# frosinastojanovska/image-captioning

Measured on AMD Instinct MI355X. Metric: captions/sec (train step) on 1024px x 32RoI x 15tok synth, higher is better.
Workload: dtype f32 (split-bf16x3 products, fp32 accumulate: 73 of 85 conv layers on the bf16 pipe, the rest and the decoder exact fp32 MFMA); 1 GPU; BASELINE configs[2] (configs[3] at 8 GPUs): frozen ResNet-101+FPN fwd + PyramidROIAlign + RoI head + v2-inject decoder fwd/bwd + AMSGrad, 1024x1024 synth images, 32 RoI/img, 15-token captions, V=10000; backbone=resnet101, images_per_gpu=2, global_batch_images=2, parallelism=dp1, stage4_blocks=22, pipeline=encoder(i+1) || decoder(i), 2 HIP streams, rccl_ranks=1

## Files before the change

### image-captioning_amd/csrc/conv_wino.hip

```cpp
#include "igemm_bf16s.h"
#include <algorithm>

namespace dcap {
namespace wino {

constexpr int NTHREADS = 256;

struct Args {
    const float* x;
    const f4* u;
    float* y;
    const float* scale;
    const float* shift;
    int N, H, W, Cin, Cout, relu;
    int gy, gx, groups;
    unsigned x_bytes, u_bytes;
};

__global__ void wino_pack_kernel(const float* __restrict__ w, float* __restrict__ u, int Cin, int Cout) {
    const long total = (long)Cin * Cout;
    const int NTG = Cout / 32, KC = Cin / 16;
    for (long idx = (long)blockIdx.x * blockDim.x + threadIdx.x; idx < total; idx += (long)gridDim.x * blockDim.x) {
        const int cin = (int)(idx % Cin), cout = (int)(idx / Cin);
        float g[3][3];
#pragma unroll
        for (int t = 0; t < 9; ++t) g[t / 3][t % 3] = w[((long)cout * 9 + t) * Cin + cin];
        float gg[4][3];
#pragma unroll
        for (int c = 0; c < 3; ++c) {
            gg[0][c] = g[0][c];
            gg[1][c] = 0.5f * (g[0][c] + g[1][c] + g[2][c]);
            gg[2][c] = 0.5f * (g[0][c] - g[1][c] + g[2][c]);
            gg[3][c] = g[2][c];
        }
        const int ntg = cout >> 5, i = cout & 31, kc = cin >> 4, kk = cin & 15, h = kk >> 3, j = (kk & 7) >> 2, e = kk & 3;
#pragma unroll
        for (int a = 0; a < 4; ++a) {
            const float r[4] = {gg[a][0], 0.5f * (gg[a][0] + gg[a][1] + gg[a][2]), 0.5f * (gg[a][0] - gg[a][1] + gg[a][2]), gg[a][2]};
#pragma unroll
            for (int b = 0; b < 4; ++b) {
                const int xi = 4 * a + b;
                u[((((long)(xi * NTG + ntg) * KC + kc) * 2 + j) * 64 + (h * 32 + i)) * 4 + e] = r[b];
            }
        }
    }
}

__global__ void wino_pack_b3_kernel(const float* __restrict__ w, unsigned short* __restrict__ u, int Cin, int Cout) {
    const long total = (long)Cin * Cout;
    const int NTG = Cout / 32, KC = Cin / 16;
    for (long idx = (long)blockIdx.x * blockDim.x + threadIdx.x; idx < total; idx += (long)gridDim.x * blockDim.x) {
        const int cin = (int)(idx % Cin), cout = (int)(idx / Cin);
        float g[3][3];
#pragma unroll
        for (int t = 0; t < 9; ++t) g[t / 3][t % 3] = w[((long)cout * 9 + t) * Cin + cin];
        float gg[4][3];
#pragma unroll
        for (int c = 0; c < 3; ++c) {
            gg[0][c] = g[0][c];
            gg[1][c] = 0.5f * (g[0][c] + g[1][c] + g[2][c]);
            gg[2][c] = 0.5f * (g[0][c] - g[1][c] + g[2][c]);
            gg[3][c] = g[2][c];
        }
        const int ntg = cout >> 5, i = cout & 31, kc = cin >> 4, kk = cin & 15, h = kk >> 3, jj = kk & 7;
#pragma unroll
        for (int a = 0; a < 4; ++a) {
            const float r[4] = {gg[a][0], 0.5f * (gg[a][0] + gg[a][1] + gg[a][2]), 0.5f * (gg[a][0] - gg[a][1] + gg[a][2]), gg[a][2]};
#pragma unroll
            for (int b = 0; b < 4; ++b) {
                const int xi = 4 * a + b;
                float x = r[b];
#pragma unroll
                for (int piece = 0; piece < 3; ++piece) {
                    const unsigned short pb = __builtin_bit_cast(unsigned short, (__bf16)x);
                    x -= __uint_as_float((unsigned)pb << 16);
                    u[((((long)(xi * NTG + ntg) * KC + kc) * 3 + piece) * 64 + (h * 32 + i)) * 8 + jj] = pb;
                }
            }
        }
    }
}

__device__ __forceinline__ unsigned img32_addr(int xi, int tile, int chunk) {
    return (unsigned)((((xi * 32 + tile) << 3) + (chunk ^ ((tile >> 1) & 7))) << 4);
}
__device__ __forceinline__ void bt_cols(const f4 (&t)[4], f4 (&v)[4]) {
    v[0] = t[0] - t[2];
    v[1] = t[1] + t[2];
    v[2] = t[2] - t[1];
    v[3] = t[1] - t[3];
}

namespace wp {
constexpr int PW = 18, NDMA = 6;
__device__ __forceinline__ int patch_index(int y, int x) { return y * PW + (x >> 1) + (PW / 2) * (x & 1); }
__device__ __forceinline__ int patch_swizzle(int y, int x) { return ((x >> 2) & 1) | (((y >> 1) & 3) << 1); }
template <int HALVES>
struct Cfg {
    static constexpr int NT = 256 * HALVES, TGY = 4 * HALVES, TGX = 8, PH = 2 * TGY + 2, NPIX = PH * PW, SLOTS = NPIX * 8;
    static constexpr int BUF = 32768 * HALVES;
    static constexpr int LDS_BYTES = 2 * BUF;
    static_assert(NDMA * NT >= SLOTS && NDMA * NT * 16 <= BUF, "patch buffer; the kernel issues the pieces three per step");
};
}

typedef unsigned u32x4 __attribute__((ext_vector_type(4)));

__device__ __forceinline__ void split8(const f4& va, const f4& vb, u32x4& p0, u32x4& p1, u32x4& p2) {
    unsigned a0, a1, a2, b0, b1, b2, c0, c1, c2, d0, d1, d2;
    split_pair(va[0], va[1], a0, a1, a2);
    split_pair(va[2], va[3], b0, b1, b2);
    split_pair(vb[0], vb[1], c0, c1, c2);
    split_pair(vb[2], vb[3], d0, d1, d2);
    p0 = u32x4{a0, b0, c0, d0};
    p1 = u32x4{a1, b1, c1, d1};
    p2 = u32x4{a2, b2, c2, d2};
}
__device__ __forceinline__ f32x16 mfma_b(const u32x4& a, const u32x4& b, const f32x16& c) {
    return __builtin_amdgcn_mfma_f32_32x32x16_bf16(__builtin_bit_cast(bf16x8, a), __builtin_bit_cast(bf16x8, b), c, 0, 0, 0);
}

template <int HALVES, bool B3>
__device__ __forceinline__ void wino_body(const Args& a) {
    using namespace wp;
    typedef Cfg<HALVES> C;
    constexpr int NT64 = C::NT, SLOTS = C::SLOTS, BUF = C::BUF;
    extern __shared__ __attribute__((aligned(16))) char smem[];
    const int tid = threadIdx.x, lane = tid & 63;
    const int wave = __builtin_amdgcn_readfirstlane(tid >> 6);
    const int wa = wave & 3, th = wave >> 2;
    const int gpi = a.gy * a.gx;
    const int NTG = a.Cout >> 5, KC = a.Cin >> 4, KP = a.Cin >> 5;
    const int total = a.groups * NTG;
    const __amdgpu_buffer_rsrc_t rsrc = __builtin_amdgcn_make_buffer_rsrc(const_cast<float*>(a.x), 0, (int)a.x_bytes, 0x00020000);

    int nb, img, gyi, gxi;
    unsigned doff[NDMA];
    const f4* ubase;
    unsigned ubyte3;
    auto setup = [&](int item) {
        const int bid = xcd_remap(item, total);
        nb = bid / a.groups;
        const int g = bid - nb * a.groups;
        img = g / gpi;
        const int gr = g - img * gpi;
        gyi = gr / a.gx;
        gxi = gr - gyi * a.gx;
#pragma unroll
        for (int n = 0; n < NDMA; ++n) {
            const int s = n * NT64 + tid, pq = s >> 3, py = pq / PW, rem = pq - py * PW;
            const int px = rem < PW / 2 ? 2 * rem : 2 * (rem - PW / 2) + 1;
            const int iy = gyi * 2 * C::TGY - 1 + py, ix = gxi * 2 * C::TGX - 1 + px;
            const bool in = s < SLOTS && (unsigned)iy < (unsigned)a.H && (unsigned)ix < (unsigned)a.W;
            const int c8 = (s & 7) ^ patch_swizzle(py, px);
            doff[n] = in ? (unsigned)(((((long)img * a.H + iy) * a.W + ix) * a.Cin + 4 * c8) * 4) : kOobOffset;
        }
        ubase = a.u + lane + (((long)(4 * wa) * NTG + nb) * KC << 7);
        ubyte3 = (unsigned)((4 * wa) * NTG + nb) * (unsigned)KC * 3072u;
    };
    auto issue_dma_pieces = [&](int pair, int buf, int n0, int n1) {
#pragma unroll
        for (int n = n0; n < n1; ++n)
            __builtin_amdgcn_raw_ptr_buffer_load_lds(rsrc, (__attribute__((address_space(3))) void*)(smem + buf * BUF + (n * NT64 + wave * 64) * 16), 16,
                                                     (int)doff[n], pair * 128, 0, 0);
    };
    auto issue_dma = [&](int pair, int buf) { issue_dma_pieces(pair, buf, 0, NDMA); };
    const long ustep = (long)NTG * KC << 7;
    auto load_u_part = [&](f4 (&dst)[4][2], int kc, int b0, int b1) {
#pragma unroll
        for (int b = b0; b < b1; ++b) {
            const f4* p = ubase + b * ustep + ((long)kc << 7);
            dst[b][0] = p[0];
            dst[b][1] = p[64];
        }
    };
    auto load_u = [&](f4 (&dst)[4][2], int kc) { load_u_part(dst, kc, 0, 4); };
    const __amdgpu_buffer_rsrc_t rsrc_u = __builtin_amdgcn_make_buffer_rsrc(const_cast<f4*>(a.u), 0, (int)a.u_bytes, 0x00020000);
    const unsigned ustep3 = (unsigned)NTG * KC * 3 * 1024u;
    auto load_u3 = [&](u32x4 (&dst)[3], int kc, int b) {
        const unsigned so = __builtin_amdgcn_readfirstlane(ubyte3 + (unsigned)b * ustep3 + (unsigned)kc * 3072u);
        dst[0] = __builtin_bit_cast(u32x4, buf_f4s(rsrc_u, (unsigned)lane * 16u, so));
        dst[1] = __builtin_bit_cast(u32x4, buf_f4s(rsrc_u, (unsigned)lane * 16u, so + 1024u));
        dst[2] = __builtin_bit_cast(u32x4, buf_f4s(rsrc_u, (unsigned)lane * 16u, so + 2048u));
    };

    const int fi = lane & 31, fh = lane >> 5;
    const int tile = 32 * th + fi, tyl = tile >> 3, txl = tile & 7;
    const int r1 = (wa == 0) ? 0 : (wa == 2 ? 2 : 1), r2 = (wa == 0 || wa == 1) ? 2 : (wa == 2 ? 1 : 3);
    const float sgn = (wa == 1) ? 1.f : -1.f;
    unsigned paddr[2][4];
#pragma unroll
    for (int rr = 0; rr < 2; ++rr)
#pragma unroll
        for (int c = 0; c < 4; ++c) {
            const int py = 2 * tyl + (rr ? r2 : r1), px = 2 * txl + c;
            paddr[rr][c] = (unsigned)(patch_index(py, px) * 128 + (((2 * fh) ^ patch_swizzle(py, px)) << 4));
        }
    auto read_d = [&](f4 (&d)[2][4], int st) {
        const unsigned k = (unsigned)(((st & 1) << 4) ^ ((st >> 1) << 6));
#pragma unroll
        for (int rr = 0; rr < 2; ++rr)
#pragma unroll
            for (int c = 0; c < 4; ++c) d[rr][c] = *reinterpret_cast<const f4*>(smem + (paddr[rr][c] ^ k));
    };
    auto transform = [&](const f4 (&d)[2][4], f4 (&v)[4]) {
        f4 t[4];
#pragma unroll
        for (int c = 0; c < 4; ++c) t[c] = d[1][c] * sgn + d[0][c];
        bt_cols(t, v);
    };

    int item = blockIdx.x;
    if (item >= total) return;
    setup(item);
    issue_dma(0, 0);
    f4 ub[2][4][2];
    u32x4 u3[4][3];
    if constexpr (B3) {
#pragma unroll
        for (int b = 0; b < 4; ++b) load_u3(u3[b], 0, b);
    } else {
        load_u(ub[0], 0);
    }
    for (;;) {
        f32x16 acc[4];
#pragma unroll
        for (int b = 0; b < 4; ++b)
#pragma unroll
            for (int r = 0; r < 16; ++r) acc[b][r] = 0.f;
        auto pair = [&](int p, auto more_c) {
            constexpr bool more = decltype(more_c)::value;
            asm volatile("s_waitcnt vmcnt(0)" ::: "memory");
            __syncthreads();
            if constexpr (B3) {
                f4 dA[2][4], dB[2][4], t0[4], t1[4];
                u32x4 V[2][3];
                auto make_t = [&]() {
#pragma unroll
                    for (int c = 0; c < 4; ++c) {
                        t0[c] = dA[1][c] * sgn + dA[0][c];
                        t1[c] = dB[1][c] * sgn + dB[0][c];
                    }
                };
                auto prep = [&](u32x4 (&dst)[3], int b) {
                    const f4 va = b == 0 ? t0[0] - t0[2] : (b == 1 ? t0[1] + t0[2] : (b == 2 ? t0[2] - t0[1] : t0[1] - t0[3]));
                    const f4 vb = b == 0 ? t1[0] - t1[2] : (b == 1 ? t1[1] + t1[2] : (b == 2 ? t1[2] - t1[1] : t1[1] - t1[3]));
                    split8(va, vb, dst[0], dst[1], dst[2]);
                };
                read_d(dA, 0);
                read_d(dB, 1);
                make_t();
                prep(V[0], 0);
#pragma unroll
                for (int q = 0; q < 8; ++q) {
                    const int half = q >> 2, b = q & 3;
                    if (q == 1) read_d(dA, 2);
                    if (q == 2) read_d(dB, 3);
                    __builtin_amdgcn_sched_barrier(0);
                    if constexpr (more) if (q < NDMA) issue_dma_pieces(p + 1, (p + 1) & 1, q, q + 1);
                    const u32x4 (&vq)[3] = V[q & 1];
                    acc[b] = mfma_b(u3[b][0], vq[2], acc[b]);
                    acc[b] = mfma_b(u3[b][1], vq[1], acc[b]);
                    acc[b] = mfma_b(u3[b][2], vq[0], acc[b]);
                    acc[b] = mfma_b(u3[b][1], vq[0], acc[b]);
                    acc[b] = mfma_b(u3[b][0], vq[1], acc[b]);
                    acc[b] = mfma_b(u3[b][0], vq[0], acc[b]);
                    if (q == 3) make_t();
                    if (q < 7) prep(V[(q + 1) & 1], (q + 1) & 3);
                    load_u3(u3[b], min(2 * p + half + 1, KC - 1), b);
#pragma unroll
                    for (int m = 0; m < 6; ++m) {
                        __builtin_amdgcn_sched_group_barrier(0x008, 1, 0);
                        __builtin_amdgcn_sched_group_barrier(0x020, 1, 0);
                        if (q == 3) __builtin_amdgcn_sched_group_barrier(0x002, 15, 0);
                        else __builtin_amdgcn_sched_group_barrier(0x002, 9, 0);
                    }
                    __builtin_amdgcn_sched_barrier(0);
                }
#pragma unroll
                for (int rr = 0; rr < 2; ++rr)
#pragma unroll
                    for (int c = 0; c < 4; ++c) paddr[rr][c] ^= (unsigned)BUF;
                return;
            }
            f4 d[2][4], vcur[4], vnext[4];
            read_d(d, 0);
            transform(d, vcur);
#pragma unroll
            for (int st = 0; st < 4; ++st) {
                const int half = st >> 1, j = st & 1;
                if (st < 3) read_d(d, st + 1);
                __builtin_amdgcn_sched_barrier(0);
                if constexpr (more) if (st < 2) issue_dma_pieces(p + 1, (p + 1) & 1, 3 * st, 3 * st + 3);
                load_u_part(ub[half ^ 1], min(2 * p + half + 1, KC - 1), 2 * j, 2 * j + 2);
#pragma unroll
                for (int e = 0; e < 2; ++e)
#pragma unroll
                    for (int b = 0; b < 4; ++b) acc[b] = __builtin_amdgcn_mfma_f32_32x32x2f32(ub[half][b][j][e], vcur[b][e], acc[b], 0, 0, 0);
#pragma unroll
                for (int m = 0; m < 8; ++m) {
                    __builtin_amdgcn_sched_group_barrier(0x008, 1, 0);
                    __builtin_amdgcn_sched_group_barrier(0x020, 1, 0);
                }
                __builtin_amdgcn_sched_barrier(0);
                if (st < 3) transform(d, vnext);
#pragma unroll
                for (int e = 2; e < 4; ++e)
#pragma unroll
                    for (int b = 0; b < 4; ++b) acc[b] = __builtin_amdgcn_mfma_f32_32x32x2f32(ub[half][b][j][e], vcur[b][e], acc[b], 0, 0, 0);
                if (st < 3) {
#pragma unroll
                    for (int m = 0; m < 8; ++m) {
                        __builtin_amdgcn_sched_group_barrier(0x008, 1, 0);
                        __builtin_amdgcn_sched_group_barrier(0x002, 4, 0);
                    }
                }
                __builtin_amdgcn_sched_barrier(0);
                if (st < 3) {
#pragma unroll
                    for (int b = 0; b < 4; ++b) vcur[b] = vnext[b];
                }
            }
#pragma unroll
            for (int rr = 0; rr < 2; ++rr)
#pragma unroll
                for (int c = 0; c < 4; ++c) paddr[rr][c] ^= (unsigned)BUF;
        };
        for (int p = 0; p < KP - 1; ++p) pair(p, std::true_type{});
        pair(KP - 1, std::false_type{});
        if (KP & 1) {
#pragma unroll
            for (int rr = 0; rr < 2; ++rr)
#pragma unroll
                for (int c = 0; c < 4; ++c) paddr[rr][c] ^= (unsigned)BUF;
        }

        const int onb = nb, oimg = img, ogy = gyi, ogx = gxi;
        const int next = item + (int)gridDim.x;
        const int oq = tid & 7, ocout = onb * 32 + 4 * oq;
        f4 sc = (f4)(1.f), sh = (f4)(0.f);
        if (a.scale) sc = *reinterpret_cast<const f4*>(a.scale + ocout);
        if (a.shift) sh = *reinterpret_cast<const f4*>(a.shift + ocout);
        __syncthreads();
        if (next < total) {
            setup(next);
            issue_dma(0, 0);
            if constexpr (B3) {
#pragma unroll
                for (int b = 0; b < 4; ++b) load_u3(u3[b], 0, b);
            } else {
                load_u(ub[0], 0);
            }
        }
        {
            const f32x16 s0 = acc[0] + acc[1] + acc[2], s1 = acc[1] - acc[2] - acc[3];
#pragma unroll
            for (int gq = 0; gq < 4; ++gq) {
                const f4 m0 = {s0[4 * gq], s0[4 * gq + 1], s0[4 * gq + 2], s0[4 * gq + 3]};
                const f4 m1 = {s1[4 * gq], s1[4 * gq + 1], s1[4 * gq + 2], s1[4 * gq + 3]};
                *reinterpret_cast<f4*>(smem + BUF + th * 32768 + img32_addr(2 * wa, fi, 2 * gq + fh)) = m0;
                *reinterpret_cast<f4*>(smem + BUF + th * 32768 + img32_addr(2 * wa + 1, fi, 2 * gq + fh)) = m1;
            }
        }
        __syncthreads();
        {
            const int oth = tid >> 8, ti = (tid >> 3) & 31;
            f4 sv[4][2];
#pragma unroll
            for (int r = 0; r < 4; ++r)
#pragma unroll
                for (int qx = 0; qx < 2; ++qx) sv[r][qx] = *reinterpret_cast<const f4*>(smem + BUF + oth * 32768 + img32_addr(2 * r + qx, ti, oq));
            const int otile = 32 * oth + ti, ty = ogy * C::TGY + (otile >> 3), tx = ogx * C::TGX + (otile & 7), cout = ocout;
#pragma unroll
            for (int qx = 0; qx < 2; ++qx) {
                const f4 o[2] = {sv[0][qx] + sv[1][qx] + sv[2][qx], sv[1][qx] - sv[2][qx] - sv[3][qx]};
#pragma unroll
                for (int pr = 0; pr < 2; ++pr) {
                    f4 val = o[pr] * sc + sh;
                    if (a.relu) val = f4{fmaxf(val[0], 0.f), fmaxf(val[1], 0.f), fmaxf(val[2], 0.f), fmaxf(val[3], 0.f)};
                    if (2 * ty + pr < a.H && 2 * tx + qx < a.W)
                        *reinterpret_cast<f4*>(a.y + (((long)oimg * a.H + 2 * ty + pr) * a.W + 2 * tx + qx) * a.Cout + cout) = val;
                }
            }
        }
        if (next >= total) break;
        item = next;
    }
}

__global__ __launch_bounds__(512, 1) void wino64_kernel(Args a) { wino_body<2, false>(a); }
__global__ __launch_bounds__(256, 2) void wino32_kernel(Args a) { wino_body<1, false>(a); }
__global__ __launch_bounds__(512, 1) void wino64b_kernel(Args a) { wino_body<2, true>(a); }
__global__ __launch_bounds__(256, 2) void wino32b_kernel(Args a) { wino_body<1, true>(a); }

}

static bool wino_shape_ok(const dc_conv_desc* d, const void* u) {
    return u != nullptr && d->math == DC_MATH_F32 && d->kh == 3 && d->kw == 3 && d->stride == 1 && d->pad_t == 1 && d->pad_l == 1 &&
           d->Ho == d->H && d->Wo == d->W && d->Cin % 32 == 0 && d->Cout % 32 == 0 && d->res_mode == 0 && d->split_k <= 1 && aligned16(d->y) &&
           aligned16(u) && (!d->scale || aligned16(d->scale)) && (!d->shift || aligned16(d->shift)) &&
           (size_t)d->N * d->H * d->W * d->Cin * sizeof(float) < (1ull << 31);
}

static bool wino_b3(const dc_conv_desc* d) { return wino_shape_ok(d, d->w_wino_b3); }
bool conv_winograd_supported(const dc_conv_desc* d) { return wino_b3(d) || wino_shape_ok(d, d->w_wino); }
bool conv_winograd_split_bf16(const dc_conv_desc* d) { return wino_b3(d); }

static int wino_force() {
    static const int force = env_int("DCAP_WINO_TILES", 0);
    return force;
}

static std::atomic<int> g_persistent_cus{-1};
static int persistent_cus() {
    int v = g_persistent_cus.load(std::memory_order_relaxed);
    if (v < 0) {
        static const int env = env_int("DCAP_WINO_CUS", kNumCU);
        v = env;
    }
    v = std::max(8, std::min(v, kNumCU));
    return v / 8 * 8;
}

int conv_winograd_tiles(const dc_conv_desc* d) {
    const int force = wino_force();
    if (force == 32 || force == 64) return force;
    if (wino_b3(d)) return 32;
    const int th = (d->H + 1) / 2, tw = (d->W + 1) / 2;
    const long items64 = (long)d->N * ((th + 7) / 8) * ((tw + 7) / 8) * (d->Cout / 32);
    return items64 >= kNumCU ? 64 : 32;
}

int conv2d_winograd(const dc_conv_desc* d, hipStream_t s) {
    wino::Args a;
    a.x = d->x;
    const bool b3 = wino_b3(d);
    a.u = b3 ? reinterpret_cast<const f4*>(d->w_wino_b3) : reinterpret_cast<const f4*>(d->w_wino);
    a.y = d->y;
    a.scale = d->scale;
    a.shift = d->shift;
    a.N = d->N; a.H = d->H; a.W = d->W; a.Cin = d->Cin; a.Cout = d->Cout; a.relu = d->relu;
    const int th = (d->H + 1) / 2, tw = (d->W + 1) / 2;
    const size_t x_bytes = (size_t)d->N * d->H * d->W * d->Cin * sizeof(float);
    DC_REQUIRE(x_bytes < (1ull << 31), DC_EINVAL, "dc_conv2d (winograd): the input tensor has %zu bytes, the kernel addresses < 2 GiB", x_bytes);
    a.x_bytes = (unsigned)x_bytes;
    a.u_bytes = (unsigned)((size_t)16 * d->Cin * d->Cout * (b3 ? 6 : 4));
    const bool big = conv_winograd_tiles(d) == 64;
    a.gy = (th + (big ? 8 : 4) - 1) / (big ? 8 : 4);
    a.gx = (tw + 7) / 8;
    a.groups = d->N * a.gy * a.gx;
    const long items = (long)a.groups * (d->Cout / 32);
    DC_REQUIRE(items < (1l << 31), DC_EINVAL, "dc_conv2d (winograd): grid too large");
    const long full = big ? kNumCU : 2 * kNumCU;
    const long slots = items >= 8 * full ? (big ? persistent_cus() : 2 * persistent_cus()) : full;
    const unsigned grid = items >= slots ? (unsigned)slots : (unsigned)std::max<long>(8, items / 8 * 8);
    if (b3 && big) {
        DC_ENSURE_DYN_LDS(wino::wino64b_kernel, wino::wp::Cfg<2>::LDS_BYTES);
        hipLaunchKernelGGL(wino::wino64b_kernel, dim3(grid), dim3(wino::wp::Cfg<2>::NT), wino::wp::Cfg<2>::LDS_BYTES, s, a);
    } else if (b3) {
        DC_ENSURE_DYN_LDS(wino::wino32b_kernel, wino::wp::Cfg<1>::LDS_BYTES);
        hipLaunchKernelGGL(wino::wino32b_kernel, dim3(grid), dim3(wino::wp::Cfg<1>::NT), wino::wp::Cfg<1>::LDS_BYTES, s, a);
    } else if (big) {
        DC_ENSURE_DYN_LDS(wino::wino64_kernel, wino::wp::Cfg<2>::LDS_BYTES);
        hipLaunchKernelGGL(wino::wino64_kernel, dim3(grid), dim3(wino::wp::Cfg<2>::NT), wino::wp::Cfg<2>::LDS_BYTES, s, a);
    } else {
        DC_ENSURE_DYN_LDS(wino::wino32_kernel, wino::wp::Cfg<1>::LDS_BYTES);
        hipLaunchKernelGGL(wino::wino32_kernel, dim3(grid), dim3(wino::wp::Cfg<1>::NT), wino::wp::Cfg<1>::LDS_BYTES, s, a);
    }
    return check_launch("dc_conv2d (winograd)");
}

}

using namespace dcap;

extern "C" size_t dc_conv2d_winograd_weight_bytes(int Cin, int Cout) {
    if (Cin <= 0 || Cout <= 0 || Cin % 32 || Cout % 32) return 0;
    return (size_t)16 * Cin * Cout * sizeof(float);
}

extern "C" int dc_conv2d_winograd_pack_f32(const float* w, float* u, int Cin, int Cout, void* stream) {
    DC_REQUIRE(w && u, DC_EINVAL, "dc_conv2d_winograd_pack: null pointer");
    DC_REQUIRE(Cin > 0 && Cout > 0 && Cin % 32 == 0 && Cout % 32 == 0, DC_EINVAL, "dc_conv2d_winograd_pack: Cin and Cout must be multiples of 32");
    DC_REQUIRE(aligned16(u), DC_EALIGN, "dc_conv2d_winograd_pack: u must be 16-byte aligned");
    const long total = (long)Cin * Cout;
    const int blocks = (int)std::min<long>((total + 255) / 256, 4096);
    hipLaunchKernelGGL(wino::wino_pack_kernel, dim3(blocks), dim3(256), 0, static_cast<hipStream_t>(stream), w, u, Cin, Cout);
    return check_launch("dc_conv2d_winograd_pack_f32");
}

extern "C" size_t dc_conv2d_winograd_b3_weight_bytes(int Cin, int Cout) {
    if (Cin <= 0 || Cout <= 0 || Cin % 32 || Cout % 32) return 0;
    return (size_t)16 * Cin * Cout * 3 * sizeof(uint16_t);
}

extern "C" int dc_conv2d_winograd_pack_b3(const float* w, uint16_t* u, int Cin, int Cout, void* stream) {
    DC_REQUIRE(w && u, DC_EINVAL, "dc_conv2d_winograd_pack_b3: null pointer");
    DC_REQUIRE(Cin > 0 && Cout > 0 && Cin % 32 == 0 && Cout % 32 == 0, DC_EINVAL, "dc_conv2d_winograd_pack_b3: Cin and Cout must be multiples of 32");
    DC_REQUIRE(aligned16(u), DC_EALIGN, "dc_conv2d_winograd_pack_b3: u must be 16-byte aligned");
    const long total = (long)Cin * Cout;
    const int blocks = (int)std::min<long>((total + 255) / 256, 4096);
    hipLaunchKernelGGL(wino::wino_pack_b3_kernel, dim3(blocks), dim3(256), 0, static_cast<hipStream_t>(stream), w, u, Cin, Cout);
    return check_launch("dc_conv2d_winograd_pack_b3");
}

extern "C" int dc_set_persistent_cus(int n) {
    DC_REQUIRE(n == 0 || (n >= 8 && n <= kNumCU), DC_EINVAL, "dc_set_persistent_cus: 0 (default: DCAP_WINO_CUS or all 256) or 8..256, got %d", n);
    dcap::g_persistent_cus.store(n == 0 ? -1 : n, std::memory_order_relaxed);
    return DC_OK;
}

extern "C" int dc_get_persistent_cus(void) { return dcap::persistent_cus(); }
```

Baseline: 11310 captions/s.

## Add 64-output-channel items to split-bf16 Winograd 32-tile kernel

```diff
diff --git a/image-captioning_amd/csrc/conv_wino.hip b/image-captioning_amd/csrc/conv_wino.hip
--- a/image-captioning_amd/csrc/conv_wino.hip
+++ b/image-captioning_amd/csrc/conv_wino.hip
@@ -120,8 +120,9 @@
     return __builtin_amdgcn_mfma_f32_32x32x16_bf16(__builtin_bit_cast(bf16x8, a), __builtin_bit_cast(bf16x8, b), c, 0, 0, 0);
 }
 
-template <int HALVES, bool B3>
+template <int HALVES, bool B3, int NCH = 1>
 __device__ __forceinline__ void wino_body(const Args& a) {
+    static_assert(NCH == 1 || (NCH == 2 && HALVES == 1 && B3), "64-channel items: the split-bf16 32-tile kernel only");
     using namespace wp;
     typedef Cfg<HALVES> C;
     constexpr int NT64 = C::NT, SLOTS = C::SLOTS, BUF = C::BUF;
@@ -131,7 +132,7 @@
     const int wa = wave & 3, th = wave >> 2;
     const int gpi = a.gy * a.gx;
     const int NTG = a.Cout >> 5, KC = a.Cin >> 4, KP = a.Cin >> 5;
-    const int total = a.groups * NTG;
+    const int total = a.groups * (NTG / NCH);
     const __amdgpu_buffer_rsrc_t rsrc = __builtin_amdgcn_make_buffer_rsrc(const_cast<float*>(a.x), 0, (int)a.x_bytes, 0x00020000);
 
     int nb, img, gyi, gxi;
@@ -156,7 +157,7 @@
             doff[n] = in ? (unsigned)(((((long)img * a.H + iy) * a.W + ix) * a.Cin + 4 * c8) * 4) : kOobOffset;
         }
         ubase = a.u + lane + (((long)(4 * wa) * NTG + nb) * KC << 7);
-        ubyte3 = (unsigned)((4 * wa) * NTG + nb) * (unsigned)KC * 3072u;
+        ubyte3 = (unsigned)((4 * wa) * NTG + NCH * nb) * (unsigned)KC * 3072u;
     };
     auto issue_dma_pieces = [&](int pair, int buf, int n0, int n1) {
 #pragma unroll
@@ -177,8 +178,8 @@
     auto load_u = [&](f4 (&dst)[4][2], int kc) { load_u_part(dst, kc, 0, 4); };
     const __amdgpu_buffer_rsrc_t rsrc_u = __builtin_amdgcn_make_buffer_rsrc(const_cast<f4*>(a.u), 0, (int)a.u_bytes, 0x00020000);
     const unsigned ustep3 = (unsigned)NTG * KC * 3 * 1024u;
-    auto load_u3 = [&](u32x4 (&dst)[3], int kc, int b) {
-        const unsigned so = __builtin_amdgcn_readfirstlane(ubyte3 + (unsigned)b * ustep3 + (unsigned)kc * 3072u);
+    auto load_u3 = [&](u32x4 (&dst)[3], int kc, int b, int hc) {
+        const unsigned so = __builtin_amdgcn_readfirstlane(ubyte3 + (unsigned)b * ustep3 + (unsigned)(hc * KC + kc) * 3072u);
         dst[0] = __builtin_bit_cast(u32x4, buf_f4s(rsrc_u, (unsigned)lane * 16u, so));
         dst[1] = __builtin_bit_cast(u32x4, buf_f4s(rsrc_u, (unsigned)lane * 16u, so + 1024u));
         dst[2] = __builtin_bit_cast(u32x4, buf_f4s(rsrc_u, (unsigned)lane * 16u, so + 2048u));
@@ -216,23 +217,107 @@
     issue_dma(0, 0);
     f4 ub[2][4][2];
     u32x4 u3[4][3];
+    u32x4 w0[2][2], w1[2], w2[2];
+    auto load_piece = [&](u32x4& dst, int kc, int b, int hc, int piece) {
+        const unsigned so = __builtin_amdgcn_readfirstlane(ubyte3 + (unsigned)b * ustep3 + (unsigned)(hc * KC + kc) * 3072u + (unsigned)piece * 1024u);
+        dst = __builtin_bit_cast(u32x4, buf_f4s(rsrc_u, (unsigned)lane * 16u, so));
+    };
+    auto load_u3_first = [&]() {
+        if constexpr (NCH == 2) {
+#pragma unroll
+            for (int hc = 0; hc < 2; ++hc) {
+                load_piece(w0[0][hc], 0, 0, hc, 0);
+                load_piece(w1[hc], 0, 0, hc, 1);
+                load_piece(w2[hc], 0, 0, hc, 2);
+                load_piece(w0[1][hc], 0, 1, hc, 0);
+            }
+        } else {
+#pragma unroll
+            for (int b = 0; b < 4; ++b) load_u3(u3[b], 0, b, 0);
+        }
+    };
     if constexpr (B3) {
-#pragma unroll
-        for (int b = 0; b < 4; ++b) load_u3(u3[b], 0, b);
+        load_u3_first();
     } else {
         load_u(ub[0], 0);
     }
     for (;;) {
-        f32x16 acc[4];
-#pragma unroll
-        for (int b = 0; b < 4; ++b)
-#pragma unroll
-            for (int r = 0; r < 16; ++r) acc[b][r] = 0.f;
+        f32x16 acc[NCH][4];
+#pragma unroll
+        for (int hc = 0; hc < NCH; ++hc)
+#pragma unroll
+            for (int b = 0; b < 4; ++b)
+#pragma unroll
+                for (int r = 0; r < 16; ++r) acc[hc][b][r] = 0.f;
         auto pair = [&](int p, auto more_c) {
             constexpr bool more = decltype(more_c)::value;
             asm volatile("s_waitcnt vmcnt(0)" ::: "memory");
             __syncthreads();
-            if constexpr (B3) {
+            if constexpr (B3 && NCH == 2) {
+                f4 t0[4], t1[4];
+                u32x4 V[2][3];
+                auto fetch_col = [&](int hf, int c) {
+                    const unsigned ka = (unsigned)(hf << 6), kb = ka ^ 16u;
+                    const f4 a0 = *reinterpret_cast<const f4*>(smem + (paddr[0][c] ^ ka));
+                    const f4 a1 = *reinterpret_cast<const f4*>(smem + (paddr[1][c] ^ ka));
+                    const f4 b0 = *reinterpret_cast<const f4*>(smem + (paddr[0][c] ^ kb));
+                    const f4 b1 = *reinterpret_cast<const f4*>(smem + (paddr[1][c] ^ kb));
+                    t0[c] = a1 * sgn + a0;
+                    t1[c] = b1 * sgn + b0;
+                };
+                auto prep = [&](u32x4 (&dst)[3], int b) {
+                    const f4 va = b == 0 ? t0[0] - t0[2] : (b == 1 ? t0[1] + t0[2] : (b == 2 ? t0[2] - t0[1] : t0[1] - t0[3]));
+                    const f4 vb = b == 0 ? t1[0] - t1[2] : (b == 1 ? t1[1] + t1[2] : (b == 2 ? t1[2] - t1[1] : t1[1] - t1[3]));
+                    split8(va, vb, dst[0], dst[1], dst[2]);
+                };
+                fetch_col(0, 0);
+                fetch_col(0, 2);
+                prep(V[0], 0);
+#pragma unroll
+                for (int q = 0; q < 8; ++q) {
+                    const int b = q & 3;
+                    __builtin_amdgcn_sched_barrier(0);
+                    if constexpr (more) if (q < NDMA) issue_dma_pieces(p + 1, (p + 1) & 1, q, q + 1);
+                    const u32x4 (&vq)[3] = V[q & 1];
+                    const int kc1 = min(2 * p + ((q + 1) >> 2), KC - 1), kc2 = min(2 * p + ((q + 2) >> 2), KC - 1);
+#pragma unroll
+                    for (int hc = 0; hc < 2; ++hc) acc[hc][b] = mfma_b(w0[q & 1][hc], vq[2], acc[hc][b]);
+#pragma unroll
+                    for (int hc = 0; hc < 2; ++hc) acc[hc][b] = mfma_b(w1[hc], vq[1], acc[hc][b]);
+#pragma unroll
+                    for (int hc = 0; hc < 2; ++hc) acc[hc][b] = mfma_b(w2[hc], vq[0], acc[hc][b]);
+#pragma unroll
+                    for (int hc = 0; hc < 2; ++hc) load_piece(w2[hc], kc1, (q + 1) & 3, hc, 2);
+#pragma unroll
+                    for (int hc = 0; hc < 2; ++hc) acc[hc][b] = mfma_b(w1[hc], vq[0], acc[hc][b]);
+#pragma unroll
+                    for (int hc = 0; hc < 2; ++hc) load_piece(w1[hc], kc1, (q + 1) & 3, hc, 1);
+#pragma unroll
+                    for (int hc = 0; hc < 2; ++hc) acc[hc][b] = mfma_b(w0[q & 1][hc], vq[1], acc[hc][b]);
+#pragma unroll
+                    for (int hc = 0; hc < 2; ++hc) acc[hc][b] = mfma_b(w0[q & 1][hc], vq[0], acc[hc][b]);
+#pragma unroll
+                    for (int hc = 0; hc < 2; ++hc) load_piece(w0[q & 1][hc], kc2, (q + 2) & 3, hc, 0);
+                    if (q == 0) fetch_col(0, 1);
+                    if (q == 1) { fetch_col(0, 3); fetch_col(1, 0); }
+                    if (q == 2) fetch_col(1, 2);
+                    if (q == 3) fetch_col(1, 1);
+                    if (q == 4) fetch_col(1, 3);
+                    if (q < 7) prep(V[(q + 1) & 1], (q + 1) & 3);
+#pragma unroll
+                    for (int m = 0; m < 12; ++m) {
+                        __builtin_amdgcn_sched_group_barrier(0x008, 1, 0);
+                        __builtin_amdgcn_sched_group_barrier(0x020, 1, 0);
+                        __builtin_amdgcn_sched_group_barrier(0x002, 6, 0);
+                    }
+                    __builtin_amdgcn_sched_barrier(0);
+                }
+#pragma unroll
+                for (int rr = 0; rr < 2; ++rr)
+#pragma unroll
+                    for (int c = 0; c < 4; ++c) paddr[rr][c] ^= (unsigned)BUF;
+                return;
+            } else if constexpr (B3) {
                 f4 dA[2][4], dB[2][4], t0[4], t1[4];
                 u32x4 V[2][3];
                 auto make_t = [&]() {
@@ -259,15 +344,15 @@
                     __builtin_amdgcn_sched_barrier(0);
                     if constexpr (more) if (q < NDMA) issue_dma_pieces(p + 1, (p + 1) & 1, q, q + 1);
                     const u32x4 (&vq)[3] = V[q & 1];
-                    acc[b] = mfma_b(u3[b][0], vq[2], acc[b]);
-                    acc[b] = mfma_b(u3[b][1], vq[1], acc[b]);
-                    acc[b] = mfma_b(u3[b][2], vq[0], acc[b]);
-                    acc[b] = mfma_b(u3[b][1], vq[0], acc[b]);
-                    acc[b] = mfma_b(u3[b][0], vq[1], acc[b]);
-                    acc[b] = mfma_b(u3[b][0], vq[0], acc[b]);
+                    acc[0][b] = mfma_b(u3[b][0], vq[2], acc[0][b]);
+                    acc[0][b] = mfma_b(u3[b][1], vq[1], acc[0][b]);
+                    acc[0][b] = mfma_b(u3[b][2], vq[0], acc[0][b]);
+                    acc[0][b] = mfma_b(u3[b][1], vq[0], acc[0][b]);
+                    acc[0][b] = mfma_b(u3[b][0], vq[1], acc[0][b]);
+                    acc[0][b] = mfma_b(u3[b][0], vq[0], acc[0][b]);
                     if (q == 3) make_t();
                     if (q < 7) prep(V[(q + 1) & 1], (q + 1) & 3);
-                    load_u3(u3[b], min(2 * p + half + 1, KC - 1), b);
+                    load_u3(u3[b], min(2 * p + half + 1, KC - 1), b, 0);
 #pragma unroll
                     for (int m = 0; m < 6; ++m) {
                         __builtin_amdgcn_sched_group_barrier(0x008, 1, 0);
@@ -296,7 +381,7 @@
 #pragma unroll
                 for (int e = 0; e < 2; ++e)
 #pragma unroll
-                    for (int b = 0; b < 4; ++b) acc[b] = __builtin_amdgcn_mfma_f32_32x32x2f32(ub[half][b][j][e], vcur[b][e], acc[b], 0, 0, 0);
+                    for (int b = 0; b < 4; ++b) acc[0][b] = __builtin_amdgcn_mfma_f32_32x32x2f32(ub[half][b][j][e], vcur[b][e], acc[0][b], 0, 0, 0);
 #pragma unroll
                 for (int m = 0; m < 8; ++m) {
                     __builtin_amdgcn_sched_group_barrier(0x008, 1, 0);
@@ -307,7 +392,7 @@
 #pragma unroll
                 for (int e = 2; e < 4; ++e)
 #pragma unroll
-                    for (int b = 0; b < 4; ++b) acc[b] = __builtin_amdgcn_mfma_f32_32x32x2f32(ub[half][b][j][e], vcur[b][e], acc[b], 0, 0, 0);
+                    for (int b = 0; b < 4; ++b) acc[0][b] = __builtin_amdgcn_mfma_f32_32x32x2f32(ub[half][b][j][e], vcur[b][e], acc[0][b], 0, 0, 0);
                 if (st < 3) {
 #pragma unroll
                     for (int m = 0; m < 8; ++m) {
@@ -337,49 +422,55 @@
 
         const int onb = nb, oimg = img, ogy = gyi, ogx = gxi;
         const int next = item + (int)gridDim.x;
-        const int oq = tid & 7, ocout = onb * 32 + 4 * oq;
-        f4 sc = (f4)(1.f), sh = (f4)(0.f);
-        if (a.scale) sc = *reinterpret_cast<const f4*>(a.scale + ocout);
-        if (a.shift) sh = *reinterpret_cast<const f4*>(a.shift + ocout);
+        const int oq = tid & 7, ocout = onb * (32 * NCH) + 4 * oq;
+        f4 sc[NCH], sh[NCH];
+#pragma unroll
+        for (int hc = 0; hc < NCH; ++hc) {
+            sc[hc] = a.scale ? *reinterpret_cast<const f4*>(a.scale + ocout + 32 * hc) : (f4)(1.f);
+            sh[hc] = a.shift ? *reinterpret_cast<const f4*>(a.shift + ocout + 32 * hc) : (f4)(0.f);
+        }
         __syncthreads();
         if (next < total) {
             setup(next);
             issue_dma(0, 0);
             if constexpr (B3) {
-#pragma unroll
-                for (int b = 0; b < 4; ++b) load_u3(u3[b], 0, b);
+                load_u3_first();
             } else {
                 load_u(ub[0], 0);
             }
         }
-        {
-            const f32x16 s0 = acc[0] + acc[1] + acc[2], s1 = acc[1] - acc[2] - acc[3];
-#pragma unroll
-            for (int gq = 0; gq < 4; ++gq) {
-                const f4 m0 = {s0[4 * gq], s0[4 * gq + 1], s0[4 * gq + 2], s0[4 * gq + 3]};
-                const f4 m1 = {s1[4 * gq], s1[4 * gq + 1], s1[4 * gq + 2], s1[4 * gq + 3]};
-                *reinterpret_cast<f4*>(smem + BUF + th * 32768 + img32_addr(2 * wa, fi, 2 * gq + fh)) = m0;
-                *reinterpret_cast<f4*>(smem + BUF + th * 32768 + img32_addr(2 * wa + 1, fi, 2 * gq + fh)) = m1;
-            }
-        }
-        __syncthreads();
-        {
-            const int oth = tid >> 8, ti = (tid >> 3) & 31;
-            f4 sv[4][2];
-#pragma unroll
-            for (int r = 0; r < 4; ++r)
-#pragma unroll
-                for (int qx = 0; qx < 2; ++qx) sv[r][qx] = *reinterpret_cast<const f4*>(smem + BUF + oth * 32768 + img32_addr(2 * r + qx, ti, oq));
-            const int otile = 32 * oth + ti, ty = ogy * C::TGY + (otile >> 3), tx = ogx * C::TGX + (otile & 7), cout = ocout;
-#pragma unroll
-            for (int qx = 0; qx < 2; ++qx) {
-                const f4 o[2] = {sv[0][qx] + sv[1][qx] + sv[2][qx], sv[1][qx] - sv[2][qx] - sv[3][qx]};
-#pragma unroll
-                for (int pr = 0; pr < 2; ++pr) {
-                    f4 val = o[pr] * sc + sh;
-                    if (a.relu) val = f4{fmaxf(val[0], 0.f), fmaxf(val[1], 0.f), fmaxf(val[2], 0.f), fmaxf(val[3], 0.f)};
-                    if (2 * ty + pr < a.H && 2 * tx + qx < a.W)
-                        *reinterpret_cast<f4*>(a.y + (((long)oimg * a.H + 2 * ty + pr) * a.W + 2 * tx + qx) * a.Cout + cout) = val;
+#pragma unroll
+        for (int hc = 0; hc < NCH; ++hc) {
+            if (hc) __syncthreads();
+            {
+                const f32x16 s0 = acc[hc][0] + acc[hc][1] + acc[hc][2], s1 = acc[hc][1] - acc[hc][2] - acc[hc][3];
+#pragma unroll
+                for (int gq = 0; gq < 4; ++gq) {
+                    const f4 m0 = {s0[4 * gq], s0[4 * gq + 1], s0[4 * gq + 2], s0[4 * gq + 3]};
+                    const f4 m1 = {s1[4 * gq], s1[4 * gq + 1], s1[4 * gq + 2], s1[4 * gq + 3]};
+                    *reinterpret_cast<f4*>(smem + BUF + th * 32768 + img32_addr(2 * wa, fi, 2 * gq + fh)) = m0;
+                    *reinterpret_cast<f4*>(smem + BUF + th * 32768 + img32_addr(2 * wa + 1, fi, 2 * gq + fh)) = m1;
+                }
+            }
+            __syncthreads();
+            {
+                const int oth = tid >> 8, ti = (tid >> 3) & 31;
+                f4 sv[4][2];
+#pragma unroll
+                for (int r = 0; r < 4; ++r)
+#pragma unroll
+                    for (int qx = 0; qx < 2; ++qx) sv[r][qx] = *reinterpret_cast<const f4*>(smem + BUF + oth * 32768 + img32_addr(2 * r + qx, ti, oq));
+                const int otile = 32 * oth + ti, ty = ogy * C::TGY + (otile >> 3), tx = ogx * C::TGX + (otile & 7), cout = ocout + 32 * hc;
+#pragma unroll
+                for (int qx = 0; qx < 2; ++qx) {
+                    const f4 o[2] = {sv[0][qx] + sv[1][qx] + sv[2][qx], sv[1][qx] - sv[2][qx] - sv[3][qx]};
+#pragma unroll
+                    for (int pr = 0; pr < 2; ++pr) {
+                        f4 val = o[pr] * sc[hc] + sh[hc];
+                        if (a.relu) val = f4{fmaxf(val[0], 0.f), fmaxf(val[1], 0.f), fmaxf(val[2], 0.f), fmaxf(val[3], 0.f)};
+                        if (2 * ty + pr < a.H && 2 * tx + qx < a.W)
+                            *reinterpret_cast<f4*>(a.y + (((long)oimg * a.H + 2 * ty + pr) * a.W + 2 * tx + qx) * a.Cout + cout) = val;
+                    }
                 }
             }
         }
@@ -391,7 +482,10 @@
 __global__ __launch_bounds__(512, 1) void wino64_kernel(Args a) { wino_body<2, false>(a); }
 __global__ __launch_bounds__(256, 2) void wino32_kernel(Args a) { wino_body<1, false>(a); }
 __global__ __launch_bounds__(512, 1) void wino64b_kernel(Args a) { wino_body<2, true>(a); }
-__global__ __launch_bounds__(256, 2) void wino32b_kernel(Args a) { wino_body<1, true>(a); }
+template <int NCH>
+__global__ __launch_bounds__(256, 2) void wino32b_kernel(Args a) { wino_body<1, true, NCH>(a); }
+template __global__ void wino32b_kernel<1>(Args);
+template __global__ void wino32b_kernel<2>(Args);
 
 }
 
@@ -429,6 +523,20 @@
     const int th = (d->H + 1) / 2, tw = (d->W + 1) / 2;
     const long items64 = (long)d->N * ((th + 7) / 8) * ((tw + 7) / 8) * (d->Cout / 32);
     return items64 >= kNumCU ? 64 : 32;
+}
+
+static int wino_cout_force() {
+    static const int force = env_int("DCAP_WINO_COUT", 0);
+    return force;
+}
+
+static int conv_winograd_cout(const dc_conv_desc* d) {
+    if (!wino_b3(d) || conv_winograd_tiles(d) != 32 || d->Cout % 64) return 32;
+    const int force = wino_cout_force();
+    if (force == 32 || force == 64) return force;
+    const int th = (d->H + 1) / 2, tw = (d->W + 1) / 2;
+    const long items = (long)d->N * ((th + 3) / 4) * ((tw + 7) / 8) * (d->Cout / 64);
+    return items >= 2 * kNumCU ? 64 : 32;
 }
 
 int conv2d_winograd(const dc_conv_desc* d, hipStream_t s) {
@@ -449,17 +557,22 @@
     a.gy = (th + (big ? 8 : 4) - 1) / (big ? 8 : 4);
     a.gx = (tw + 7) / 8;
     a.groups = d->N * a.gy * a.gx;
-    const long items = (long)a.groups * (d->Cout / 32);
+    const bool wide = b3 && !big && conv_winograd_cout(d) == 64;
+    const long items = (long)a.groups * (d->Cout / (wide ? 64 : 32));
     DC_REQUIRE(items < (1l << 31), DC_EINVAL, "dc_conv2d (winograd): grid too large");
-    const long full = big ? kNumCU : 2 * kNumCU;
-    const long slots = items >= 8 * full ? (big ? persistent_cus() : 2 * persistent_cus()) : full;
+    const int per_cu = big ? 1 : 2;
+    const long full = (long)per_cu * kNumCU;
+    const long slots = items >= 8 * full ? per_cu * persistent_cus() : full;
     const unsigned grid = items >= slots ? (unsigned)slots : (unsigned)std::max<long>(8, items / 8 * 8);
     if (b3 && big) {
         DC_ENSURE_DYN_LDS(wino::wino64b_kernel, wino::wp::Cfg<2>::LDS_BYTES);
         hipLaunchKernelGGL(wino::wino64b_kernel, dim3(grid), dim3(wino::wp::Cfg<2>::NT), wino::wp::Cfg<2>::LDS_BYTES, s, a);
+    } else if (wide) {
+        DC_ENSURE_DYN_LDS((&wino::wino32b_kernel<2>), wino::wp::Cfg<1>::LDS_BYTES);
+        hipLaunchKernelGGL((wino::wino32b_kernel<2>), dim3(grid), dim3(wino::wp::Cfg<1>::NT), wino::wp::Cfg<1>::LDS_BYTES, s, a);
     } else if (b3) {
-        DC_ENSURE_DYN_LDS(wino::wino32b_kernel, wino::wp::Cfg<1>::LDS_BYTES);
-        hipLaunchKernelGGL(wino::wino32b_kernel, dim3(grid), dim3(wino::wp::Cfg<1>::NT), wino::wp::Cfg<1>::LDS_BYTES, s, a);
+        DC_ENSURE_DYN_LDS((&wino::wino32b_kernel<1>), wino::wp::Cfg<1>::LDS_BYTES);
+        hipLaunchKernelGGL((wino::wino32b_kernel<1>), dim3(grid), dim3(wino::wp::Cfg<1>::NT), wino::wp::Cfg<1>::LDS_BYTES, s, a);
     } else if (big) {
         DC_ENSURE_DYN_LDS(wino::wino64_kernel, wino::wp::Cfg<2>::LDS_BYTES);
         hipLaunchKernelGGL(wino::wino64_kernel, dim3(grid), dim3(wino::wp::Cfg<2>::NT), wino::wp::Cfg<2>::LDS_BYTES, s, a);
```

Result: faster. 11560 captions/s (median of 6 runs) (+2.2%).
